# trzy/FasterRCNN

Measured on AMD Instinct MI355X. Metric: images/sec (600x1000) Faster-RCNN VGG-16 inference, higher is better.
Workload: dtype f32 (float32 tensors and accumulation; 15 GEMM layers in the f32x3 split-operand emulation = two fp16 terms per block-scaled operand, three fp16 MFMAs per product; 0 in f32x6 = three bf16 terms, six bf16 MFMAs; the other 2 on exact-f32 MFMA; strict exact-f32 everywhere: config.strict_f32_images_per_

## Files before the change

### fasterrcnn_amd/_native.py

```python
import ctypes as C
import os

_HERE = os.path.dirname(os.path.abspath(__file__))
LIB_PATH = os.environ.get("FRCNN_LIB_PATH") or os.path.join(_HERE, "csrc", "libfrcnn_hip.so")

OK = 0
ABI_VERSION = 21
ERRORS = {0: "FRCNN_OK", -1: "FRCNN_EINVAL", -2: "FRCNN_EHIP", -3: "FRCNN_ENOMEM",
          -4: "FRCNN_EUNSUPPORTED", -5: "FRCNN_ENODEVICE"}
RELU = 1
POOL2 = 2
NUM_KCLASS = 11
KCLASS_NAMES = ("conv3x3_mfma", "conv3x3_c3", "linear_mfma", "proposals", "roi_pool", "other", "winograd_transforms",
                "winograd_gemm", "winograd_x6_transforms", "winograd_x6_gemm", "winograd_x3f")

SYMBOLS = (
    "frcnn_abi_version", "frcnn_error_string", "frcnn_last_hip_error", "frcnn_device_count",
    "frcnn_anchors", "frcnn_pack_conv3x3", "frcnn_pack_conv3x3_c3", "frcnn_pack_fc_chw_to_hwc",
    "frcnn_pack_stack_rows", "frcnn_conv3x3_c3", "frcnn_conv3x3_c3_cmax", "frcnn_conv3x3_workspace_bytes", "frcnn_conv3x3_nhwc",
    "frcnn_maxpool2x2_nhwc",
    "frcnn_linear_workspace_bytes", "frcnn_linear", "frcnn_softmax_rows", "frcnn_rpn_proposals",
    "frcnn_nms", "frcnn_roi_pool", "frcnn_roi_pool_x3t", "frcnn_detections", "frcnn_ctx_create", "frcnn_ctx_create_proposals", "frcnn_ctx_destroy",
    "frcnn_ctx_bytes", "frcnn_vgg16_forward", "frcnn_ctx_tensor", "frcnn_ctx_timing_enable",
    "frcnn_ctx_timing_read",
    "frcnn_output_block_layout", "frcnn_stream_depend", "frcnn_ctx_submit_stats", "frcnn_predict_submit", "frcnn_streams_share_queue",
# ... 1 lines not shown
    "frcnn_maxpool3x3_s2_nhwc", "frcnn_spatial_mean_nhwc", "frcnn_resnet_forward", "frcnn_rpn_targets",
    "frcnn_preprocess_workspace_bytes", "frcnn_preprocess",
    "frcnn_conv3x3_uses_winograd", "frcnn_resnet_block_uses_winograd", "frcnn_pack_conv3x3_winograd",
    "frcnn_pack_conv3x3_winograd_taps", "frcnn_conv3x3_winograd_workspace_bytes",
    "frcnn_conv3x3_nhwc_winograd",
    "frcnn_conv3x3_uses_winograd_fused", "frcnn_resnet_block_uses_winograd_fused", "frcnn_pack_conv3x3_winograd_fused", "frcnn_pack_conv3x3_winograd_fused_taps",
    "frcnn_conv3x3_nhwc_winograd_fused",
    "frcnn_roi_align", "frcnn_roi_align_backward",
    "frcnn_x6t_record_bytes", "frcnn_split_rows_x6t", "frcnn_gemm_x6t_workspace_bytes", "frcnn_gemm_x6t", "frcnn_split_pixels_x6t", "frcnn_split_patches3x3_x6t",
    "frcnn_conv3x3_uses_winograd_x6", "frcnn_conv3x3_winograd_x6_pack_bytes", "frcnn_pack_conv3x3_winograd_x6",
    "frcnn_conv3x3_winograd_x6_workspace_bytes", "frcnn_conv3x3_nhwc_winograd_x6",
    "frcnn_pixel_absmax", "frcnn_split_pixels_x3t", "frcnn_split_patches3x3_x3t",
    "frcnn_x3t_blob_bytes", "frcnn_pack_rows_x3t", "frcnn_conv3x3_winograd_x3_pack_bytes", "frcnn_pack_conv3x3_winograd_x3",
    "frcnn_conv3x3_winograd_x3_workspace_bytes", "frcnn_conv3x3_nhwc_winograd_x3",
    "frcnn_conv3x3_winograd_x3_fused_workspace_bytes", "frcnn_conv3x3_nhwc_winograd_x3_fused", "frcnn_conv3x3_nhwc_winograd_x3_chain",
    "frcnn_x3t_record_bytes", "frcnn_rows_scale_x3t", "frcnn_split_rows_x3t", "frcnn_gemm_x3t_workspace_bytes", "frcnn_gemm_x3t",
    "frcnn_conv3x3_nhwc_winograd_fused_maps", "frcnn_ctx_create_backbone", "frcnn_resnet_backbone", "frcnn_resnet_forward_features", "frcnn_resnet_rpn_roipool", "frcnn_ctx_create_head", "frcnn_resnet_head",
    "frcnn_label_proposals", "frcnn_gather_rows", "frcnn_rpn_loss", "frcnn_detector_loss",
    "frcnn_gemm_tn_math", "frcnn_conv3x3_wgrad_math", "frcnn_conv_wgrad_math", "frcnn_bottleneck_backward_workspace_bytes", "frcnn_bottleneck_backward",
    "frcnn_gemm_tn_workspace_bytes", "frcnn_gemm_tn", "frcnn_conv3x3_wgrad_workspace_bytes", "frcnn_conv3x3_wgrad",
    "frcnn_pack_conv3x3_dgrad", "frcnn_relu_backward", "frcnn_dropout", "frcnn_dropout_relu_backward", "frcnn_add_inplace", "frcnn_maxpool2x2_backward",
    "frcnn_roi_pool_backward_workspace_bytes", "frcnn_roi_pool_backward", "frcnn_transpose", "frcnn_sgd_step", "frcnn_sgd_step_fold",
    "frcnn_conv_wgrad_workspace_bytes", "frcnn_conv_wgrad", "frcnn_conv_dgrad_workspace_bytes", "frcnn_conv_dgrad", "frcnn_conv_dgrad_math",
    "frcnn_pack_conv_dgrad", "frcnn_scale_rows", "frcnn_bn_scale_shift", "frcnn_spatial_mean_backward",
    "frcnn_ops_roi_align", "frcnn_ops_roi_align_backward", "frcnn_ops_roi_pool", "frcnn_ops_roi_pool_backward",
    "frcnn_ops_nms_workspace_bytes", "frcnn_ops_nms",
    "frcnn_ops_ms_roi_align", "frcnn_ops_ms_roi_align_workspace_bytes", "frcnn_ops_ms_roi_align_backward",
    "frcnn_ops_half_run", "frcnn_ops_roi_align_16", "frcnn_ops_roi_align_backward_16", "frcnn_ops_roi_pool_16",
    "frcnn_ops_roi_pool_backward_16", "frcnn_ops_ms_roi_align_16", "frcnn_ops_ms_roi_align_backward_16",
    "frcnn_ops_ps_roi_pool", "frcnn_ops_ps_roi_pool_backward", "frcnn_ops_ps_roi_align", "frcnn_ops_ps_roi_align_backward",
    "frcnn_ops_ps_roi_pool_16", "frcnn_ops_ps_roi_pool_backward_16", "frcnn_ops_ps_roi_align_16", "frcnn_ops_ps_roi_align_backward_16",
# ... 259 lines not shown
    "frcnn_split_pixels_x3t": (C.c_int, [_vp, _vp, _vp, _vp, _i, _i, _i, _i, _i, _i, _vp]),
    "frcnn_split_patches3x3_x3t": (C.c_int, [_vp, _vp, _vp, _vp, _i, _i, _i, _i, _i, _i, _vp]),
    "frcnn_x3t_blob_bytes": (C.c_size_t, [_i, _i, _i]),
    "frcnn_pack_rows_x3t": (C.c_int, [_vp, _i, _sz, _vp, _i, _i, _i, _i, _vp]),
    "frcnn_conv3x3_winograd_x3_pack_bytes": (C.c_size_t, [_i, _i]),
    "frcnn_pack_conv3x3_winograd_x3": (C.c_int, [_vp, _vp, _i, _i, _vp]),
    "frcnn_conv3x3_winograd_x3_workspace_bytes": (C.c_size_t, [_i, _i, _i, _i, _i]),
    "frcnn_conv3x3_nhwc_winograd_x3": (C.c_int, [_vp, _vp, _vp, _vp, _i, _i, _i, _i, _i, _u, _vp, _sz, _vp]),
    "frcnn_conv3x3_winograd_x3_fused_workspace_bytes": (C.c_size_t, [_i, _i, _i]),
    "frcnn_conv3x3_nhwc_winograd_x3_fused": (C.c_int, [_vp, _vp, _vp, _vp, _i, _i, _i, _i, _i, _u, _vp, _sz, _vp]),
    "frcnn_conv3x3_nhwc_winograd_x3_chain": (C.c_int, [_vp, _vp, _vp, _vp, _i, _i, _i, _i, _i, _u, _i, _vp, _sz, _vp, _vp, _vp]),
    "frcnn_x3t_record_bytes": (C.c_size_t, [_i, _i]),
    "frcnn_rows_scale_x3t": (C.c_int, [_vp, _i, _sz, _vp, _i, _i, _i, _i, _vp]),
    "frcnn_split_rows_x3t": (C.c_int, [_vp, _i, _sz, _vp, _vp, _i, _i, _i, _i, _vp]),
    "frcnn_gemm_x3t_workspace_bytes": (C.c_size_t, [_i, _i, _i, _i]),
    "frcnn_gemm_x3t": (C.c_int, [_vp, _vp, _i, _sz, _sz, _vp, _vp, _i, _sz, _sz, _vp, _vp, _vp, _i, _sz, _i, _i, _i, _i, _u, _vp, _sz, _vp]),
    "frcnn_ctx_create_backbone": (C.c_int, [C.POINTER(C.c_void_p), _i, _i, _i]),
    "frcnn_ctx_create_head": (C.c_int, [C.POINTER(C.c_void_p), _i]),
    "frcnn_resnet_rpn_roipool": (C.c_int, [_vp, C.POINTER(ResNetWeights), C.POINTER(ForwardParams), _vp, _i, _i, _vp, _vp, _vp, _vp, _vp, _vp]),
    "frcnn_resnet_head": (C.c_int, [_vp, C.POINTER(ResNetWeights), C.POINTER(ForwardParams), _vp, _i, _vp, _vp, _vp]),
    "frcnn_conv3x3_nhwc_winograd_fused_maps": (C.c_int, [_vp, _vp, _vp, _vp, _i, _i, _i, _i, _i, _u, _vp]),
    "frcnn_label_proposals": (C.c_int, [_vp, _vp, _i, _vp, _vp, _i, _i, _f, _f, C.POINTER(C.c_float), C.POINTER(C.c_float),
                                        _vp, _vp, _vp, _vp, _vp, _vp]),
    "frcnn_gather_rows": (C.c_int, [_vp, _vp, _i, _i, _vp, _vp]),
    "frcnn_rpn_loss": (C.c_int, [_vp, _i, _i, _vp, _i, _vp, _vp, _vp, _vp]),
    "frcnn_detector_loss": (C.c_int, [_vp, _vp, _vp, _vp, _i, _i, _vp, _vp, _i, _vp]),
    "frcnn_gemm_tn_workspace_bytes": (C.c_size_t, [_i, _i, _i]),
    "frcnn_gemm_tn": (C.c_int, [_vp, _i, _vp, _i, _vp, _i, _i, _i, _i, _vp, _sz, _vp]),
    "frcnn_gemm_tn_math": (C.c_int, [_vp, _i, _vp, _i, _vp, _i, _i, _i, _i, _i, _vp, _sz, _vp]),
    "frcnn_conv3x3_wgrad_math": (C.c_int, [_vp, _vp, _vp, _i, _i, _i, _i, _i, _vp, _sz, _vp]),
# ... 104 lines not shown
```

### fasterrcnn_amd/csrc/api.hip

```cpp
#include "common.h"
#include <algorithm>
#include <cmath>
#include <cstring>
#include <string>
#include <vector>
#include <new>

namespace frcnn {

static thread_local std::string g_hip_error;
void set_hip_error(hipError_t e) { g_hip_error = hipGetErrorString(e); }

static size_t align_up(size_t v, size_t a) { return (v + a - 1) / a * a; }

struct EventRec { int cls; hipEvent_t start, stop; };

}

using namespace frcnn;

struct frcnn_ctx {
    int max_h = 0, max_w = 0, max_rois = 0, max_images = 0;
    int max_fh = 0, max_fw = 0, a_cap = 0, pre_cap = 0;
    void* slab = nullptr;
// ... 265 lines not shown
                         void* stream)
{
    if (!d_a || !d_inv_scale) return FRCNN_EINVAL;
    return launch_rows_scale_x3t(d_a, lda, a_batch_floats, d_inv_scale, rows, rows_padded, K, batches, as_stream(stream));
}

int frcnn_split_rows_x3t(const float* d_a, int lda, size_t a_batch_floats, const float* d_inv_scale, void* d_rec, int rows, int rows_padded,
                         int K, int batches, void* stream)
{
    if (!d_a || !d_rec || !d_inv_scale) return FRCNN_EINVAL;
    return launch_split_rows_x3t(d_a, lda, a_batch_floats, d_inv_scale, d_rec, rows, rows_padded, K, batches, as_stream(stream));
}

size_t frcnn_gemm_x3t_workspace_bytes(int M, int N, int K, int batches) { return gemm_x3t_workspace_bytes(M, N, K, batches); }

int frcnn_gemm_x3t(const void* d_a_rec, const float* d_a_inv, int a_rows, size_t a_batch_bytes, size_t a_inv_batch_floats,
                   const void* d_b_rec, const float* d_b_inv, int b_rows, size_t b_batch_bytes, size_t b_inv_batch_floats,
                   const float* d_bias, const float* d_residual, float* d_c, int ldc, size_t c_batch_floats, int M, int N, int K,
                   int batches, unsigned flags, void* d_ws, size_t ws_bytes, void* stream)
{
    return launch_gemm_x3t(d_a_rec, d_a_inv, a_rows, a_batch_bytes, a_inv_batch_floats, d_b_rec, d_b_inv, b_rows, b_batch_bytes,
                           b_inv_batch_floats, d_bias, d_residual, d_c, ldc, c_batch_floats, M, N, K, batches, flags, d_ws, ws_bytes,
                           as_stream(stream));
}

size_t frcnn_conv3x3_winograd_x3_fused_workspace_bytes(int n_maps, int H, int W)
{
    return n_maps > 0 && H > 0 && W > 0 ? conv3x3_winograd_x3_fused_workspace_bytes(n_maps, H, W) : 0;
}

int frcnn_conv3x3_nhwc_winograd_x3_fused(const float* d_x, const void* d_blob, const float* d_bias, float* d_y, int n_maps, int H, int W,
                                         int cin, int cout, unsigned flags, void* d_ws, size_t ws_bytes, void* stream)
{
    if (!d_x || !d_blob || !d_bias || !d_y) return FRCNN_EINVAL;
    return launch_conv3x3_winograd_x3_fused(d_x, d_blob, d_bias, d_y, n_maps, H, W, cin, cout, flags, d_ws, ws_bytes, as_stream(stream));
}

int frcnn_pixel_absmax(const float* d_x, float* d_cmax, long long pixels, int c, void* stream)
// ... 1038 lines not shown
    if (fc_x6t || fc_x3t) { rc = ensure_fc_records(c, s); if (rc) return rc; }
    if (fc_x3t) {
        const int rr = c->rec_rows;
        const size_t w1rec = x3t_record_bytes(4096, 49 * 512), w2rec = x3t_record_bytes(4096, 4096);
        const float* w1inv = reinterpret_cast<const float*>(reinterpret_cast<const unsigned char*>(w->fc1_w) + w1rec);
        const float* w2inv = reinterpret_cast<const float*>(reinterpret_cast<const unsigned char*>(w->fc2_w) + w2rec);
        if (p->roi_op == FRCNN_ROI_ALIGN) {
            STEP(4, launch_roi_align(c->fm, fh, fw, 512, d_props, d_counts + 2, R_, 7, 1.0f / 16.0f, p->roi_sampling_ratio, 0, c->roi_out, s));
            STEP(2, launch_rows_scale_x3t(c->roi_out, 49 * 512, 0, c->roi_inv, R_, rr, 49 * 512, 1, s));
            STEP(2, launch_split_rows_x3t(c->roi_out, 49 * 512, 0, c->roi_inv, c->roi_rec, R_, rr, 49 * 512, 1, s));
        } else {
            STEP(4, launch_roi_pool_x3t(c->fm, fh, fw, 512, d_props, d_counts + 2, R_, 7, 1.0f / 16.0f,
                                        fm_cmax_ready ? const_cast<float*>(fm_cmax_ready) : c->fm_cmax, c->roi_inv, c->roi_rec, rr, s, fm_cmax_ready != nullptr));
        }
        STEP(2, launch_gemm_x3t(c->roi_rec, c->roi_inv, rr, 0, 0, w->fc1_w, w1inv, 4096, 0, 0, w->fc1_b, nullptr, c->fc1_out, 4096, 0, R_, 4096,
                                49 * 512, 1, R, c->lin_ws, c->lin_ws_bytes, s, 0));
        STEP(2, launch_rows_scale_x3t(c->fc1_out, 4096, 0, c->fc1_inv, R_, rr, 4096, 1, s));
        STEP(2, launch_split_rows_x3t(c->fc1_out, 4096, 0, c->fc1_inv, c->fc1_rec, R_, rr, 4096, 1, s));
        STEP(2, launch_gemm_x3t(c->fc1_rec, c->fc1_inv, rr, 0, 0, w->fc2_w, w2inv, 4096, 0, 0, w->fc2_b, nullptr, c->fc2_out, 4096, 0, R_, 4096,
                                4096, 1, R, c->lin_ws, c->lin_ws_bytes, s, 2));
    } else
    if (fc_x6t) {
        const int rr = c->rec_rows;
        if (p->roi_op == FRCNN_ROI_ALIGN) {
            STEP(4, launch_roi_align(c->fm, fh, fw, 512, d_props, d_counts + 2, R_, 7, 1.0f / 16.0f, p->roi_sampling_ratio, 0, c->roi_out, s));
            STEP(2, launch_split_rows_x6t(c->roi_out, 49 * 512, 0, c->roi_rec, R_, rr, 49 * 512, 1, s));
        } else {
            STEP(4, launch_roi_pool_x6t(c->fm, fh, fw, 512, d_props, d_counts + 2, R_, 7, 1.0f / 16.0f, c->roi_rec, rr, s));
        }
        static const int fc_tiles = []() { const char* e = frcnn_knob("FRCNN_FC_TILES"); return e ? atoi(e) : 0; }();
        STEP(2, launch_gemm_x6t(c->roi_rec, rr, 0, w->fc1_w, 4096, 0, w->fc1_b, nullptr, c->fc1_out, 4096, 0, R_, 4096, 49 * 512, 1, R,
                                c->lin_ws, c->lin_ws_bytes, s, fc_tiles));
        STEP(2, launch_split_rows_x6t(c->fc1_out, 4096, 0, c->fc1_rec, R_, rr, 4096, 1, s));
        STEP(2, launch_gemm_x6t(c->fc1_rec, rr, 0, w->fc2_w, 4096, 0, w->fc2_b, nullptr, c->fc2_out, 4096, 0, R_, 4096, 4096, 1, R,
                                c->lin_ws, c->lin_ws_bytes, s, fc_tiles));
// ... 649 lines not shown
```

### fasterrcnn_amd/csrc/common.h

```cpp
#pragma once
#include <hip/hip_runtime.h>
#include <stdint.h>
#include <stddef.h>
#include <stdlib.h>
#include "../../include/frcnn_hip.h"

typedef float f32x4  __attribute__((ext_vector_type(4)));
typedef float f32x16 __attribute__((ext_vector_type(16)));

inline const char* frcnn_knob(const char* name)
{
#ifdef FRCNN_EXPERIMENT_KNOBS
    return getenv(name);
#else
    (void)name;
    return nullptr;
#endif
}

namespace frcnn {

void set_hip_error(hipError_t e);

inline int check_launch() {
// ... 115 lines not shown
int launch_gemm_x6t_reduce(const float* ws, const float* bias, const float* residual, float* c, int ldc, size_t c_batch_floats, int M, int N,
                           int batches, int splits, int relu, hipStream_t s);
size_t x3t_record_bytes(int rows_padded, int K);
int launch_rows_scale_x3t(const float* a, int lda, size_t a_batch_floats, float* inv_scale, int R, int rows_padded, int K, int batches,
                          hipStream_t s);
int launch_split_rows_x3t(const float* a, int lda, size_t a_batch_floats, const float* inv_scale, void* rec, int R, int rows_padded, int K,
                          int batches, hipStream_t s);
int launch_split_pixels_x3t(const float* x, const float* cmax, void* rec, float* inv, int N, int H, int W, int C, int stride, int rows_padded,
                            hipStream_t s);
int launch_split_patches3x3_x3t(const float* x, const float* cmax, void* rec, float* inv, int N, int H, int W, int C, int stride,
                                int rows_padded, hipStream_t s);
size_t gemm_x3t_workspace_bytes(int M, int N, int K, int batches);
int launch_gemm_x3t(const void* a_rec, const float* a_inv, int a_rows, size_t a_batch_bytes, size_t a_inv_batch, const void* b_rec,
                    const float* b_inv, int b_rows, size_t b_batch_bytes, size_t b_inv_batch, const float* bias, const float* residual,
                    float* c, int ldc, size_t c_batch_floats, int M, int N, int K, int batches, unsigned flags, void* ws, size_t ws_bytes,
                    hipStream_t s, int tiles_mode = -1);
size_t x3t_blob_bytes(int rows_padded, int K, int batches);
int launch_pack_rows_x3t(const float* a, int lda, size_t a_batch_floats, void* blob, int R, int rows_padded, int K, int batches, hipStream_t s);
int launch_pixel_absmax(const float* x, float* cmax, long long pixels, int C, hipStream_t s);
size_t conv3x3_winograd_x3_pack_bytes(int cout, int cin);
int launch_pack_conv3x3_winograd_x3(const float* u_f32, void* ublob, int cout, int cin, hipStream_t s);
size_t conv3x3_winograd_x3_workspace_bytes(int N, int H, int W, int cin, int cout);
int winograd_x3_plan(int N, int H, int W, int cin, int cout, unsigned flags, void* ws, size_t ws_bytes, void** V, float** vinv, float** cmax,
                     float** M, void** G, size_t* g_bytes);
int launch_winograd_x3_input(const float* x, float* cmax, void* vrec, float* vinv, int N, int H, int W, int cin, hipStream_t s,
                             const float* cmax_ready = nullptr);
int launch_winograd_x3_gemm(const void* vrec, const float* vinv, const void* ublob, float* M, int N, int H, int W, int cin, int cout, void* gws,
                            size_t gws_bytes, hipStream_t s);
int launch_conv3x3_winograd_x3(const float* x, const void* ublob, const float* b, float* y, int N, int H, int W, int cin, int cout,
                               unsigned flags, void* ws, size_t ws_bytes, hipStream_t s,
                               const float* cmax_ready = nullptr, float* cmax_out = nullptr);
// ... 106 lines not shown
```

### fasterrcnn_amd/csrc/gemm_x3t.hip

```cpp
#include "x3t.h"

namespace frcnn {

typedef _Float16 hx_f16x8 __attribute__((ext_vector_type(8)));

#ifndef HX_ABLATE
#define HX_ABLATE 0
#endif
__global__ __launch_bounds__(256)
void rows_scale_x3t_kernel(const float* __restrict__ a, int lda, size_t a_batch, float* __restrict__ inv_scale, int R, int rows_padded,
                           int K, int batches)
{
    const int lane = threadIdx.x & 63;
    const long long wave = (long long)blockIdx.x * 4 + (threadIdx.x >> 6);
    if (wave >= (long long)batches * rows_padded) return;
    const int row = (int)(wave % rows_padded), batch = (int)(wave / rows_padded);
    float mx = 0.f;
    if (row < R) {
        const float* src = a + (size_t)batch * a_batch + (size_t)row * lda;
        for (int k = 4 * lane; k < K; k += 256) {
            const f32x4 v = *reinterpret_cast<const f32x4*>(src + k);
            mx = fmaxf(fmaxf(mx, fmaxf(fabsf(v[0]), fabsf(v[1]))), fmaxf(fabsf(v[2]), fabsf(v[3])));
        }
    }
// ... 168 lines not shown
    const unsigned char* b;
    const float* a_inv;
    const float* b_inv;
    float* c;
    float* ws;
    const float* bias;
    const float* residual;
    size_t a_batch, b_batch, c_batch;
    size_t a_inv_batch, b_inv_batch;
    int a_rbt, b_rbt;
    int M, N, ldc;
    int nchunks, chunks_per_split, splits, batches;
    int mtiles, ntiles;
    int relu;
    int total;
};

template <int WTM, int WTN, int WVM, int WVN, int NSUB>
struct HxCfg {
    static constexpr int NW = WVM * WVN, THREADS = 64 * NW;
    static constexpr int ARB = WVM * WTM, BRB = WVN * WTN;
    static constexpr int BM = 32 * ARB, BN = 32 * BRB;
    static constexpr int A_BYTES = ARB * HX_RB, B_BYTES = BRB * HX_RB;
    static constexpr int STAGE1 = A_BYTES + B_BYTES;
    static constexpr int STAGE = NSUB * STAGE1;
    static constexpr int NBUF = NSUB == 1 ? 3 : 2;
    static constexpr int DIST = NBUF - 1;
    static constexpr size_t LDS_BYTES = NBUF * (size_t)STAGE;
    static constexpr int NPA = ARB * 2, NPB = BRB * 2, NP = NPA + NPB;
    static constexpr int PPW = (NSUB * NP + NW - 1) / NW;
};

typedef __attribute__((address_space(3))) void* hx_lds_ptr;

template <int WTM, int WTN, int WVM, int WVN, int NSUB>
__global__ __launch_bounds__(64 * WVM * WVN, 2)
void gemm_x3t_kernel(const HxParams p)
{
    using C = HxCfg<WTM, WTN, WVM, WVN, NSUB>;
    extern __shared__ __attribute__((aligned(16))) unsigned char smem_hx[];
    const int tid = threadIdx.x, lane = tid & 63;
    const int wave = __builtin_amdgcn_readfirstlane(tid >> 6);
    const int wm = wave / WVN, wn = wave % WVN;

    int bid = blockIdx.x;
    {
        const int q = p.total >> 3, r = p.total & 7, xcd = bid & 7, idx = bid >> 3;
        bid = (xcd < r ? xcd * (q + 1) : r * (q + 1) + (xcd - r) * q) + idx;
    }
    const int nt = bid % p.ntiles;
    int t = bid / p.ntiles;
    const int mt = t % p.mtiles;
    t /= p.mtiles;
// ... 10 lines not shown
    const unsigned char* bg = p.b + (size_t)batch * p.b_batch + (size_t)nt * C::B_BYTES + (size_t)c_begin * b_chunk + lane * 16;

    auto issue_stage = [&](int s, int buf) {
        const unsigned char* as = ag + (size_t)s * NSUB * a_chunk;
        const unsigned char* bs = bg + (size_t)s * NSUB * b_chunk;
        unsigned char* ldsb = smem_hx + buf * C::STAGE;
#pragma unroll
        for (int i = 0; i < C::PPW; ++i) {
            int q = wave + C::NW * i;
            q = q < NSUB * C::NP ? q : NSUB * C::NP - 1;
            const int sub = q / C::NP, r = q - sub * C::NP;
            const unsigned char* src = r < C::NPA ? as + sub * a_chunk + r * HX_PIECE : bs + sub * b_chunk + (r - C::NPA) * HX_PIECE;
            __builtin_amdgcn_global_load_lds(src, (hx_lds_ptr)(ldsb + sub * C::STAGE1 + r * HX_PIECE), 16, 0, 0);
        }
    };
    f32x16 acc[WTM][WTN];
#pragma unroll
    for (int i = 0; i < WTM; ++i)
#pragma unroll
        for (int j = 0; j < WTN; ++j)
#pragma unroll
            for (int r = 0; r < 16; ++r) acc[i][j][r] = 0.f;

    hx_f16x8 ah[WTM], al[WTM], bh[WTN], bl[WTN];
#pragma unroll
    for (int i = 0; i < WTM; ++i)
#pragma unroll
        for (int e = 0; e < 8; ++e) al[i][e] = (_Float16)0.f;
#pragma unroll
    for (int j = 0; j < WTN; ++j)
#pragma unroll
        for (int e = 0; e < 8; ++e) bh[j][e] = (_Float16)0.f;

#ifndef HX_NO_SCHED
#define HX_NO_SCHED 0
#endif
#define HX_SGB(mask, n) __builtin_amdgcn_sched_group_barrier(mask, n, 0)
#define HX_TERM(A, B)                                                                                  \
    _Pragma("unroll") for (int i = 0; i < WTM; ++i)                                                     \
        _Pragma("unroll") for (int j = 0; j < WTN; ++j)                                                 \
            if (!(HX_ABLATE & 2)) acc[i][j] = __builtin_amdgcn_mfma_f32_32x32x16_f16(B[j], A[i], acc[i][j], 0, 0, 0);

#ifdef HX_CLOCKS
    unsigned long long clk0 = 0, real0 = 0, clk1 = 0, real1 = 0;
    const unsigned long long real_entry = __builtin_amdgcn_s_memrealtime();
#endif
    if (nst > 0) {
        issue_stage(0, 0);
        if (C::DIST == 2) issue_stage(nst > 1 ? 1 : 0, 1);
        asm volatile("s_waitcnt vmcnt(%0)" ::"n"((C::DIST - 1) * C::PPW) : "memory");
        __builtin_amdgcn_s_barrier();
        int cur = 0;
        const int a_off = wm * WTM * HX_RB + lane * 16;
        const int b_off = C::A_BYTES + wn * WTN * HX_RB + lane * 16;
#ifdef HX_CLOCKS
        clk0 = __builtin_readcyclecounter(); real0 = __builtin_amdgcn_s_memrealtime();
#endif
        for (int s = 0; s < nst; ++s) {
            const int nxt = C::NBUF == 3 ? (cur == 0 ? 2 : cur - 1) : (cur ^ 1);
#pragma unroll
            for (int sub = 0; sub < NSUB; ++sub) {
// ... 43 lines not shown
        HX_TERM(al, bh)
        asm volatile("s_waitcnt vmcnt(0)" ::: "memory");
    }
#undef HX_TERM
#undef HX_SGB

    const bool direct = p.splits == 1;
    float* dst;
    int ldd;
    if (direct) { dst = p.c + (size_t)batch * p.c_batch; ldd = p.ldc; }
    else        { dst = p.ws + ((size_t)split * p.batches + batch) * (size_t)p.M * p.N; ldd = p.N; }
    const int m_base = mt * C::BM + 32 * WTM * wm + (lane & 31);
    const int n_base = nt * C::BN + 32 * WTN * wn + 4 * (lane >> 5);
    const float* ainv = p.a_inv + (size_t)batch * p.a_inv_batch;
    const float* binv = p.b_inv + (size_t)batch * p.b_inv_batch;
#pragma unroll
    for (int i = 0; i < WTM; ++i) {
        const int m = m_base + 32 * i;
        if (m >= p.M) continue;
        const float sa = ainv[m];
        float* row = dst + (size_t)m * ldd;
#pragma unroll
        for (int j = 0; j < WTN; ++j) {
#pragma unroll
            for (int g = 0; g < 4; ++g) {
                const int n = n_base + 32 * j + 8 * g;
                if (n >= p.N) continue;
                const f32x4 sb = *reinterpret_cast<const f32x4*>(binv + n);
                f32x4 v;
#pragma unroll
                for (int e = 0; e < 4; ++e) v[e] = (acc[i][j][4 * g + e] * sa) * sb[e];
                if (direct && p.bias != nullptr) v = v + *reinterpret_cast<const f32x4*>(p.bias + n);
                if (direct && p.residual != nullptr)
                    v = v + *reinterpret_cast<const f32x4*>(p.residual + (size_t)batch * p.c_batch + (size_t)m * ldd + n);
                if (direct && p.relu) {
#pragma unroll
                    for (int e = 0; e < 4; ++e) v[e] = fmaxf(v[e], 0.f);
                }
                if (HX_ABLATE & 4) asm volatile("" ::"v"(v));
                else *reinterpret_cast<f32x4*>(row + n) = v;
            }
        }
    }
#ifdef HX_CLOCKS
    if (lane == 0 && p.ws != nullptr) {
        const unsigned long long real_exit = __builtin_amdgcn_s_memrealtime();
        float* o = p.ws + ((size_t)blockIdx.x * C::NW + wave) * 8;
        o[0] = (float)(clk1 - clk0); o[1] = (float)(real1 - real0); o[2] = (float)(real0 - real_entry); o[3] = (float)(real_exit - real1);
        o[4] = (float)nst; o[5] = (float)(real_entry & 0xFFFFFF); o[6] = (float)(real_exit & 0xFFFFFF); o[7] = 1.0f;
    }
#endif
}

size_t x3t_record_bytes(int rows_padded, int K) { return (size_t)(K / 16) * (rows_padded / 32) * HX_RB; }

int launch_rows_scale_x3t(const float* a, int lda, size_t a_batch_floats, float* inv_scale, int R, int rows_padded, int K, int batches,
                          hipStream_t s)
// ... 81 lines not shown
    return pl;
}

size_t gemm_x3t_workspace_bytes(int M, int N, int K, int batches)
{
    if (!gemm_x6t_shape_ok(M, N, K, batches)) return 0;
    size_t need = 0;
    for (int mode = 0; mode < 3; ++mode) {
        const HxPlan pl = plan_gemm_x3t(M, N, K, batches, mode);
        const size_t b = pl.splits > 1 ? (size_t)pl.splits * batches * M * N * sizeof(float) : 0;
        if (b > need) need = b;
    }
    return need;
}

int launch_gemm_x3t(const void* a_rec, const float* a_inv, int a_rows, size_t a_batch_bytes, size_t a_inv_batch, const void* b_rec,
                    const float* b_inv, int b_rows, size_t b_batch_bytes, size_t b_inv_batch, const float* bias, const float* residual,
                    float* c, int ldc, size_t c_batch_floats, int M, int N, int K, int batches, unsigned flags, void* ws, size_t ws_bytes,
                    hipStream_t s, int tiles_mode)
{
    if (!gemm_x6t_shape_ok(M, N, K, batches)) return FRCNN_EUNSUPPORTED;
    if (!a_rec || !b_rec || !a_inv || !b_inv || !c || a_rows % 320 != 0 || a_rows < M || b_rows % 256 != 0 || b_rows < N || ldc < N ||
        ldc % 4 != 0)
        return FRCNN_EINVAL;
    const HxPlan pl = plan_gemm_x3t(M, N, K, batches, tiles_mode);
    if (pl.splits > 1 && (ws == nullptr || ws_bytes < (size_t)pl.splits * batches * M * N * sizeof(float))) return FRCNN_EINVAL;
    HxParams p;
    p.a = static_cast<const unsigned char*>(a_rec);
    p.b = static_cast<const unsigned char*>(b_rec);
    p.a_inv = a_inv; p.b_inv = b_inv;
    p.c = c;
    p.ws = static_cast<float*>(ws);
    p.bias = bias;
    p.residual = residual;
    p.a_batch = a_batch_bytes; p.b_batch = b_batch_bytes; p.c_batch = c_batch_floats;
    p.a_inv_batch = a_inv_batch; p.b_inv_batch = b_inv_batch;
    p.a_rbt = a_rows / 32; p.b_rbt = b_rows / 32;
    p.M = M; p.N = N; p.ldc = ldc;
    p.nchunks = K / 16; p.chunks_per_split = pl.chunks_per_split; p.splits = pl.splits; p.batches = batches;
    p.mtiles = pl.mtiles; p.ntiles = pl.ntiles;
    p.relu = (flags & FRCNN_RELU) ? 1 : 0;
    const long long total = (long long)pl.mtiles * pl.ntiles * batches * pl.splits;
    if (total > 0x7fffffffLL) return FRCNN_EINVAL;
    p.total = (int)total;
    static const int env_nsub = []() { const char* e = frcnn_knob("FRCNN_HX_NSUB"); return e ? atoi(e) : 0; }();
    const int last = p.nchunks - (pl.splits - 1) * pl.chunks_per_split;
    const bool even = pl.chunks_per_split % 2 == 0 && last % 2 == 0;
    const int nsub = !even ? 1 : (env_nsub == 1 || env_nsub == 2) ? env_nsub : (pl.chunks_per_split >= 64 ? 2 : 1);
#define HX_LAUNCH(TM, TN, VM, VN, NS)                                                                          \
    do {                                                                                                      \
        using C = HxCfg<TM, TN, VM, VN, NS>;                                                                    \
        auto kern = gemm_x3t_kernel<TM, TN, VM, VN, NS>;                                                        \
        FRCNN_MAX_LDS_ONCE(kern, C::LDS_BYTES);                                                                 \
        hipLaunchKernelGGL(kern, dim3((unsigned)total), dim3(C::THREADS), C::LDS_BYTES, s, p);                  \
    } while (0)
    if (pl.cfg == 1) { if (nsub == 2) HX_LAUNCH(5, 1, 1, 4, 2); else HX_LAUNCH(5, 1, 1, 4, 1); }
    else             { if (nsub == 2) HX_LAUNCH(5, 2, 2, 4, 2); else HX_LAUNCH(5, 2, 2, 4, 1); }
#undef HX_LAUNCH
    int rc = check_launch();
    if (rc || pl.splits == 1) return rc;
    return launch_gemm_x6t_reduce(static_cast<const float*>(ws), bias, residual, c, ldc, c_batch_floats, M, N, batches, pl.splits, p.relu, s);
}

}
```

### include/frcnn_hip.h

```cpp
#ifndef FRCNN_HIP_H
#define FRCNN_HIP_H

#include <stddef.h>
#include <stdint.h>

#ifdef __cplusplus
extern "C" {
#endif

#define FRCNN_OK            0
#define FRCNN_EINVAL       -1
#define FRCNN_EHIP         -2
#define FRCNN_ENOMEM       -3
#define FRCNN_EUNSUPPORTED -4
#define FRCNN_ENODEVICE    -5

#define FRCNN_ABI_VERSION 21

#define FRCNN_RELU   1u
#define FRCNN_POOL2  2u
#define FRCNN_X3G_WSPLIT 0x800u

int         frcnn_abi_version(void);
const char* frcnn_error_string(int code);
const char* frcnn_last_hip_error(void);
int         frcnn_device_count(void);

int frcnn_anchors(int image_h, int image_w, int fh, int fw, int feature_pixels,
                  float* d_anchor_map, float* d_valid_map, void* stream);

size_t frcnn_preprocess_workspace_bytes(int H, int W, int out_h, int out_w);
int frcnn_preprocess(const unsigned char* d_rgb, int H, int W, int out_h, int out_w, int bgr_order,
                     int horizontal_flip, float scaling, const float* means, const float* stds,
                     float* d_out, unsigned char* d_out_u8, void* d_ws, size_t ws_bytes, void* stream);

// ... 61 lines not shown
int frcnn_conv3x3_nhwc_winograd_x3_fused(const float* d_x, const void* d_blob, const float* d_bias, float* d_y, int n_maps, int H, int W,
                                         int cin, int cout, unsigned flags, void* d_ws, size_t ws_bytes, void* stream);
int frcnn_conv3x3_nhwc_winograd_x3_chain(const float* d_x, const void* d_blob, const float* d_bias, float* d_y, int n_maps, int H, int W, int cin,
                                         int cout, unsigned flags, int one_launch, void* d_ws, size_t ws_bytes, const float* d_cmax_in,
                                         float* d_cmax_out, void* stream);
size_t frcnn_x3t_record_bytes(int rows_padded, int K);
int frcnn_rows_scale_x3t(const float* d_a, int lda, size_t a_batch_floats, float* d_inv_scale, int rows, int rows_padded, int K, int batches,
                         void* stream);
int frcnn_split_rows_x3t(const float* d_a, int lda, size_t a_batch_floats, const float* d_inv_scale, void* d_rec, int rows, int rows_padded,
                         int K, int batches, void* stream);
size_t frcnn_gemm_x3t_workspace_bytes(int M, int N, int K, int batches);
int frcnn_gemm_x3t(const void* d_a_rec, const float* d_a_inv, int a_rows, size_t a_batch_bytes, size_t a_inv_batch_floats,
                   const void* d_b_rec, const float* d_b_inv, int b_rows, size_t b_batch_bytes, size_t b_inv_batch_floats,
                   const float* d_bias, const float* d_residual, float* d_c, int ldc, size_t c_batch_floats, int M, int N, int K,
                   int batches, unsigned flags, void* d_ws, size_t ws_bytes, void* stream);

int frcnn_split_pixels_x6t(const float* d_x, void* d_rec, int N, int H, int W, int C, int stride, int rows_padded, void* stream);
int frcnn_conv3x3_uses_winograd_x6(int cin, int cout);
size_t frcnn_conv3x3_winograd_x6_pack_bytes(int cout, int cin);
int frcnn_pack_conv3x3_winograd_x6(const float* d_w_oihw, const float* d_row_scale, void* d_u_rec, int cout, int cin, void* stream);
size_t frcnn_conv3x3_winograd_x6_workspace_bytes(int n_maps, int H, int W, int cin, int cout);
int frcnn_conv3x3_nhwc_winograd_x6(const float* d_x, const void* d_u_rec, const float* d_bias, float* d_y, int n_maps, int H, int W, int cin,
                                   int cout, unsigned flags, void* d_ws, size_t ws_bytes, void* stream);
int frcnn_split_patches3x3_x6t(const float* d_x, void* d_rec, int N, int H, int W, int C, int stride, int rows_padded, void* stream);
int frcnn_maxpool2x2_nhwc(const float* d_x, float* d_y, int H, int W, int c, void* stream);

int frcnn_fold_bn_pack(const float* d_w_oihw, const float* d_gamma, const float* d_beta,
                       const float* d_mean, const float* d_var, float eps, int cout, int cin, int ksize,
                       float* d_w_packed, float* d_b_packed, void* stream);
size_t frcnn_conv_workspace_bytes(int N, int H, int W, int cin, int cout, int ksize, int stride, int pad);
// ... 399 lines not shown
```

Measured before the change: 979.6.

## Add 16x16x32 MFMA variant of x3t GEMM with padded-tile skipping for fc1

Adds a templated path to the split-fp16 x3t GEMM kernel that uses 16x16x32 f16 MFMA instructions with per-16-row accumulators instead of the 32x32 shape. When the row count leaves the last 16-row tile of a wave empty, that tile's loads and MFMAs are skipped. The path is enabled by default for the fc1 head GEMM. fc2 keeps the old shape. The aim is to cut MFMA work wasted on padded ROI rows and possibly raise instruction throughput, at the cost of more LDS reads and a different register footprint. A plan-query API and env override are also added.

```diff
diff --git a/fasterrcnn_amd/_native.py b/fasterrcnn_amd/_native.py
--- a/fasterrcnn_amd/_native.py
+++ b/fasterrcnn_amd/_native.py
@@ -9,6 +9,7 @@
 ERRORS = {0: "FRCNN_OK", -1: "FRCNN_EINVAL", -2: "FRCNN_EHIP", -3: "FRCNN_ENOMEM",
           -4: "FRCNN_EUNSUPPORTED", -5: "FRCNN_ENODEVICE"}
 RELU = 1
+X3T_MFMA16, X3T_MFMA16_PADDED = 0x1000, 0x2000
 POOL2 = 2
 NUM_KCLASS = 11
 KCLASS_NAMES = ("conv3x3_mfma", "conv3x3_c3", "linear_mfma", "proposals", "roi_pool", "other", "winograd_transforms",
@@ -40,7 +41,7 @@
     "frcnn_x3t_blob_bytes", "frcnn_pack_rows_x3t", "frcnn_conv3x3_winograd_x3_pack_bytes", "frcnn_pack_conv3x3_winograd_x3",
     "frcnn_conv3x3_winograd_x3_workspace_bytes", "frcnn_conv3x3_nhwc_winograd_x3",
     "frcnn_conv3x3_winograd_x3_fused_workspace_bytes", "frcnn_conv3x3_nhwc_winograd_x3_fused", "frcnn_conv3x3_nhwc_winograd_x3_chain",
-    "frcnn_x3t_record_bytes", "frcnn_rows_scale_x3t", "frcnn_split_rows_x3t", "frcnn_gemm_x3t_workspace_bytes", "frcnn_gemm_x3t",
+    "frcnn_x3t_record_bytes", "frcnn_rows_scale_x3t", "frcnn_split_rows_x3t", "frcnn_gemm_x3t_workspace_bytes", "frcnn_gemm_x3t", "frcnn_gemm_x3t_plan",
     "frcnn_conv3x3_nhwc_winograd_fused_maps", "frcnn_ctx_create_backbone", "frcnn_resnet_backbone", "frcnn_resnet_forward_features", "frcnn_resnet_rpn_roipool", "frcnn_ctx_create_head", "frcnn_resnet_head",
     "frcnn_label_proposals", "frcnn_gather_rows", "frcnn_rpn_loss", "frcnn_detector_loss",
     "frcnn_gemm_tn_math", "frcnn_conv3x3_wgrad_math", "frcnn_conv_wgrad_math", "frcnn_bottleneck_backward_workspace_bytes", "frcnn_bottleneck_backward",
@@ -330,6 +331,7 @@
     "frcnn_rows_scale_x3t": (C.c_int, [_vp, _i, _sz, _vp, _i, _i, _i, _i, _vp]),
     "frcnn_split_rows_x3t": (C.c_int, [_vp, _i, _sz, _vp, _vp, _i, _i, _i, _i, _vp]),
     "frcnn_gemm_x3t_workspace_bytes": (C.c_size_t, [_i, _i, _i, _i]),
+    "frcnn_gemm_x3t_plan": (C.c_int, [_i, _i, _i, _i, _u, _vp]),
     "frcnn_gemm_x3t": (C.c_int, [_vp, _vp, _i, _sz, _sz, _vp, _vp, _i, _sz, _sz, _vp, _vp, _vp, _i, _sz, _i, _i, _i, _i, _u, _vp, _sz, _vp]),
     "frcnn_ctx_create_backbone": (C.c_int, [C.POINTER(C.c_void_p), _i, _i, _i]),
     "frcnn_ctx_create_head": (C.c_int, [C.POINTER(C.c_void_p), _i]),
diff --git a/fasterrcnn_amd/csrc/api.hip b/fasterrcnn_amd/csrc/api.hip
--- a/fasterrcnn_amd/csrc/api.hip
+++ b/fasterrcnn_amd/csrc/api.hip
@@ -303,6 +303,10 @@
 
 size_t frcnn_gemm_x3t_workspace_bytes(int M, int N, int K, int batches) { return gemm_x3t_workspace_bytes(M, N, K, batches); }
 
+static constexpr int FC1_X3T_SHAPE = 1, FC2_X3T_SHAPE = 0;
+
+static int x3t_shape_of_flags(unsigned flags) { return (flags & FRCNN_X3T_MFMA16) ? ((flags & FRCNN_X3T_MFMA16_PADDED) ? 2 : 1) : 0; }
+
 int frcnn_gemm_x3t(const void* d_a_rec, const float* d_a_inv, int a_rows, size_t a_batch_bytes, size_t a_inv_batch_floats,
                    const void* d_b_rec, const float* d_b_inv, int b_rows, size_t b_batch_bytes, size_t b_inv_batch_floats,
                    const float* d_bias, const float* d_residual, float* d_c, int ldc, size_t c_batch_floats, int M, int N, int K,
@@ -310,7 +314,12 @@
 {
     return launch_gemm_x3t(d_a_rec, d_a_inv, a_rows, a_batch_bytes, a_inv_batch_floats, d_b_rec, d_b_inv, b_rows, b_batch_bytes,
                            b_inv_batch_floats, d_bias, d_residual, d_c, ldc, c_batch_floats, M, N, K, batches, flags, d_ws, ws_bytes,
-                           as_stream(stream));
+                           as_stream(stream), -1, x3t_shape_of_flags(flags));
+}
+
+int frcnn_gemm_x3t_plan(int M, int N, int K, int batches, unsigned flags, int32_t* out7)
+{
+    return gemm_x3t_plan(M, N, K, batches, x3t_shape_of_flags(flags), -1, out7);
 }
 
 size_t frcnn_conv3x3_winograd_x3_fused_workspace_bytes(int n_maps, int H, int W)
@@ -1379,11 +1388,11 @@
                                         fm_cmax_ready ? const_cast<float*>(fm_cmax_ready) : c->fm_cmax, c->roi_inv, c->roi_rec, rr, s, fm_cmax_ready != nullptr));
         }
         STEP(2, launch_gemm_x3t(c->roi_rec, c->roi_inv, rr, 0, 0, w->fc1_w, w1inv, 4096, 0, 0, w->fc1_b, nullptr, c->fc1_out, 4096, 0, R_, 4096,
-                                49 * 512, 1, R, c->lin_ws, c->lin_ws_bytes, s, 0));
+                                49 * 512, 1, R, c->lin_ws, c->lin_ws_bytes, s, 0, FC1_X3T_SHAPE));
         STEP(2, launch_rows_scale_x3t(c->fc1_out, 4096, 0, c->fc1_inv, R_, rr, 4096, 1, s));
         STEP(2, launch_split_rows_x3t(c->fc1_out, 4096, 0, c->fc1_inv, c->fc1_rec, R_, rr, 4096, 1, s));
         STEP(2, launch_gemm_x3t(c->fc1_rec, c->fc1_inv, rr, 0, 0, w->fc2_w, w2inv, 4096, 0, 0, w->fc2_b, nullptr, c->fc2_out, 4096, 0, R_, 4096,
-                                4096, 1, R, c->lin_ws, c->lin_ws_bytes, s, 2));
+                                4096, 1, R, c->lin_ws, c->lin_ws_bytes, s, 2, FC2_X3T_SHAPE));
     } else
     if (fc_x6t) {
         const int rr = c->rec_rows;
diff --git a/fasterrcnn_amd/csrc/common.h b/fasterrcnn_amd/csrc/common.h
--- a/fasterrcnn_amd/csrc/common.h
+++ b/fasterrcnn_amd/csrc/common.h
@@ -153,7 +153,8 @@
 int launch_gemm_x3t(const void* a_rec, const float* a_inv, int a_rows, size_t a_batch_bytes, size_t a_inv_batch, const void* b_rec,
                     const float* b_inv, int b_rows, size_t b_batch_bytes, size_t b_inv_batch, const float* bias, const float* residual,
                     float* c, int ldc, size_t c_batch_floats, int M, int N, int K, int batches, unsigned flags, void* ws, size_t ws_bytes,
-                    hipStream_t s, int tiles_mode = -1);
+                    hipStream_t s, int tiles_mode = -1, int shape = 0);
+int gemm_x3t_plan(int M, int N, int K, int batches, int shape, int tiles_mode, int out[7]);
 size_t x3t_blob_bytes(int rows_padded, int K, int batches);
 int launch_pack_rows_x3t(const float* a, int lda, size_t a_batch_floats, void* blob, int R, int rows_padded, int K, int batches, hipStream_t s);
 int launch_pixel_absmax(const float* x, float* cmax, long long pixels, int C, hipStream_t s);
diff --git a/fasterrcnn_amd/csrc/gemm_x3t.hip b/fasterrcnn_amd/csrc/gemm_x3t.hip
--- a/fasterrcnn_amd/csrc/gemm_x3t.hip
+++ b/fasterrcnn_amd/csrc/gemm_x3t.hip
@@ -206,6 +206,7 @@
     int mtiles, ntiles;
     int relu;
     int total;
+    int skip_tiles;
 };
 
 template <int WTM, int WTN, int WVM, int WVN, int NSUB>
@@ -225,10 +226,11 @@
 
 typedef __attribute__((address_space(3))) void* hx_lds_ptr;
 
-template <int WTM, int WTN, int WVM, int WVN, int NSUB>
+template <int WTM, int WTN, int WVM, int WVN, int NSUB, int MF = 0>
 __global__ __launch_bounds__(64 * WVM * WVN, 2)
 void gemm_x3t_kernel(const HxParams p)
 {
+    static_assert(MF == 0 || NSUB == 2, "the 16x16x32 shape consumes two 16-k chunks per instruction");
     using C = HxCfg<WTM, WTN, WVM, WVN, NSUB>;
     extern __shared__ __attribute__((aligned(16))) unsigned char smem_hx[];
     const int tid = threadIdx.x, lane = tid & 63;
@@ -269,23 +271,34 @@
             __builtin_amdgcn_global_load_lds(src, (hx_lds_ptr)(ldsb + sub * C::STAGE1 + r * HX_PIECE), 16, 0, 0);
         }
     };
-    f32x16 acc[WTM][WTN];
-#pragma unroll
-    for (int i = 0; i < WTM; ++i)
-#pragma unroll
-        for (int j = 0; j < WTN; ++j)
+    constexpr int RT = 2 * WTM, CT = 2 * WTN;
+    f32x16 acc[MF ? 1 : WTM][MF ? 1 : WTN];
+    f32x4 acc4[MF ? RT : 1][MF ? CT : 1];
+#pragma unroll
+    for (int i = 0; i < (MF ? 1 : WTM); ++i)
+#pragma unroll
+        for (int j = 0; j < (MF ? 1 : WTN); ++j)
 #pragma unroll
             for (int r = 0; r < 16; ++r) acc[i][j][r] = 0.f;
-
-    hx_f16x8 ah[WTM], al[WTM], bh[WTN], bl[WTN];
-#pragma unroll
-    for (int i = 0; i < WTM; ++i)
+#pragma unroll
+    for (int i = 0; i < (MF ? RT : 1); ++i)
+#pragma unroll
+        for (int j = 0; j < (MF ? CT : 1); ++j)
+#pragma unroll
+            for (int r = 0; r < 4; ++r) acc4[i][j][r] = 0.f;
+
+    constexpr int TG = CT >= 4 ? 1 : 2, NG = RT / TG;
+    static_assert(RT % TG == 0, "row tiles per step");
+    hx_f16x8 ah[MF ? 2 * TG : WTM], al[MF ? 2 * TG : WTM], bh[MF ? CT : WTN], bl[MF ? CT : WTN];
+#pragma unroll
+    for (int i = 0; i < (MF ? 2 * TG : WTM); ++i)
 #pragma unroll
         for (int e = 0; e < 8; ++e) al[i][e] = (_Float16)0.f;
 #pragma unroll
-    for (int j = 0; j < WTN; ++j)
+    for (int j = 0; j < (MF ? CT : WTN); ++j)
 #pragma unroll
         for (int e = 0; e < 8; ++e) bh[j][e] = (_Float16)0.f;
+    const bool last_live = !p.skip_tiles || mt * C::BM + 32 * WTM * wm + 16 * (RT - 1) < p.M;
 
 #ifndef HX_NO_SCHED
 #define HX_NO_SCHED 0
@@ -300,6 +313,69 @@
     unsigned long long clk0 = 0, real0 = 0, clk1 = 0, real1 = 0;
     const unsigned long long real_entry = __builtin_amdgcn_s_memrealtime();
 #endif
+    if constexpr (MF == 1) {
+        if (nst > 0) {
+            issue_stage(0, 0);
+            asm volatile("s_waitcnt vmcnt(0)" ::: "memory");
+            __builtin_amdgcn_s_barrier();
+            int cur = 0;
+            const int frag = ((lane >> 5) & 1) * C::STAGE1 + ((lane >> 4) & 1) * 512 + (lane & 15) * 16;
+            const int a_off = wm * WTM * HX_RB + frag;
+            const int b_off = C::A_BYTES + wn * WTN * HX_RB + frag;
+#ifdef HX_CLOCKS
+            clk0 = __builtin_readcyclecounter(); real0 = __builtin_amdgcn_s_memrealtime();
+#endif
+#define HX_LD16(base, t, term) (*reinterpret_cast<const hx_f16x8*>((base) + ((t) >> 1) * HX_RB + ((t) & 1) * 256 + (term) * HX_PIECE))
+#define HX_READA(rt) do { ah[(rt) % (2 * TG)] = HX_LD16(at, rt, 0); al[(rt) % (2 * TG)] = HX_LD16(at, rt, 1); } while (0)
+#define HX_TILE16(rt)                                                                                                                      \
+    do {                                                                                                                                   \
+        _Pragma("unroll") for (int j = 0; j < CT; ++j)                                                                                     \
+            acc4[rt][j] = __builtin_amdgcn_mfma_f32_16x16x32_f16(bh[j], al[(rt) % (2 * TG)], acc4[rt][j], 0, 0, 0);                   \
+        _Pragma("unroll") for (int j = 0; j < CT; ++j)                                                                                     \
+            acc4[rt][j] = __builtin_amdgcn_mfma_f32_16x16x32_f16(bl[j], ah[(rt) % (2 * TG)], acc4[rt][j], 0, 0, 0);                   \
+        _Pragma("unroll") for (int j = 0; j < CT; ++j)                                                                                     \
+            acc4[rt][j] = __builtin_amdgcn_mfma_f32_16x16x32_f16(bh[j], ah[(rt) % (2 * TG)], acc4[rt][j], 0, 0, 0);                   \
+    } while (0)
+            for (int s = 0; s < nst; ++s) {
+                const unsigned char* at = smem_hx + cur * C::STAGE + a_off;
+                const unsigned char* bt = smem_hx + cur * C::STAGE + b_off;
+#pragma unroll
+                for (int j = 0; j < CT; ++j) bh[j] = HX_LD16(bt, j, 0);
+#pragma unroll
+                for (int t = 0; t < TG; ++t) HX_READA(t);
+#pragma unroll
+                for (int j = 0; j < CT; ++j) bl[j] = HX_LD16(bt, j, 1);
+                issue_stage(s + 1 < nst ? s + 1 : nst - 1, cur ^ 1);
+                __builtin_amdgcn_sched_barrier(0);
+#pragma unroll
+                for (int gi = 0; gi < NG; ++gi) {
+                    if (gi + 1 < NG) {
+#pragma unroll
+                        for (int t = 0; t < TG; ++t) {
+                            const int rt = (gi + 1) * TG + t;
+                            if (rt < RT - 1 || last_live) HX_READA(rt);
+                        }
+                    }
+#pragma unroll
+                    for (int t = 0; t < TG; ++t) {
+                        const int rt = gi * TG + t;
+                        if (rt < RT - 1 || last_live) HX_TILE16(rt);
+                    }
+                    __builtin_amdgcn_sched_barrier(0);
+                }
+                asm volatile("s_waitcnt vmcnt(0) lgkmcnt(0)" ::: "memory");
+                __builtin_amdgcn_s_barrier();
+                cur ^= 1;
+                __builtin_amdgcn_sched_barrier(0);
+            }
+#undef HX_TILE16
+#undef HX_READA
+#undef HX_LD16
+#ifdef HX_CLOCKS
+            clk1 = __builtin_readcyclecounter(); real1 = __builtin_amdgcn_s_memrealtime();
+#endif
+        }
+    } else
     if (nst > 0) {
         issue_stage(0, 0);
         if (C::DIST == 2) issue_stage(nst > 1 ? 1 : 0, 1);
@@ -373,6 +449,34 @@
     const int n_base = nt * C::BN + 32 * WTN * wn + 4 * (lane >> 5);
     const float* ainv = p.a_inv + (size_t)batch * p.a_inv_batch;
     const float* binv = p.b_inv + (size_t)batch * p.b_inv_batch;
+    if constexpr (MF == 1) {
+        const int m16 = mt * C::BM + 32 * WTM * wm + (lane & 15);
+        const int n16 = nt * C::BN + 32 * WTN * wn + 4 * (lane >> 4);
+#pragma unroll
+        for (int i = 0; i < RT; ++i) {
+            const int m = m16 + 16 * i;
+            if (m >= p.M) continue;
+            const float sa = ainv[m];
+            float* row = dst + (size_t)m * ldd;
+#pragma unroll
+            for (int j = 0; j < CT; ++j) {
+                const int n = n16 + 16 * j;
+                if (n >= p.N) continue;
+                const f32x4 sb = *reinterpret_cast<const f32x4*>(binv + n);
+                f32x4 v;
+#pragma unroll
+                for (int e = 0; e < 4; ++e) v[e] = (acc4[i][j][e] * sa) * sb[e];
+                if (direct && p.bias != nullptr) v = v + *reinterpret_cast<const f32x4*>(p.bias + n);
+                if (direct && p.residual != nullptr)
+                    v = v + *reinterpret_cast<const f32x4*>(p.residual + (size_t)batch * p.c_batch + (size_t)m * ldd + n);
+                if (direct && p.relu) {
+#pragma unroll
+                    for (int e = 0; e < 4; ++e) v[e] = fmaxf(v[e], 0.f);
+                }
+                *reinterpret_cast<f32x4*>(row + n) = v;
+            }
+        }
+    } else {
 #pragma unroll
     for (int i = 0; i < WTM; ++i) {
         const int m = m_base + 32 * i;
@@ -400,6 +504,7 @@
                 else *reinterpret_cast<f32x4*>(row + n) = v;
             }
         }
+    }
     }
 #ifdef HX_CLOCKS
     if (lane == 0 && p.ws != nullptr) {
@@ -511,10 +616,35 @@
     return need;
 }
 
+struct HxPick { int nsub, shape; };
+
+static HxPick pick_gemm_x3t(const HxPlan& pl, int nchunks, int shape)
+{
+    static const int env_nsub = []() { const char* e = frcnn_knob("FRCNN_HX_NSUB"); return e ? atoi(e) : 0; }();
+    static const int env_shape = []() { const char* e = frcnn_knob("FRCNN_HX_SHAPE"); return e ? atoi(e) : -1; }();
+    if (env_shape >= 0 && env_shape <= 2) shape = env_shape;
+    const int last = nchunks - (pl.splits - 1) * pl.chunks_per_split;
+    const bool even = pl.chunks_per_split % 2 == 0 && last % 2 == 0;
+    HxPick pk;
+    pk.shape = even && (shape == 1 || shape == 2) ? shape : 0;
+    pk.nsub = !even ? 1 : pk.shape ? 2 : (env_nsub == 1 || env_nsub == 2) ? env_nsub : (pl.chunks_per_split >= 64 ? 2 : 1);
+    return pk;
+}
+
+int gemm_x3t_plan(int M, int N, int K, int batches, int shape, int tiles_mode, int out[7])
+{
+    if (!gemm_x6t_shape_ok(M, N, K, batches)) return FRCNN_EUNSUPPORTED;
+    if (!out) return FRCNN_EINVAL;
+    const HxPlan pl = plan_gemm_x3t(M, N, K, batches, tiles_mode);
+    const HxPick pk = pick_gemm_x3t(pl, K / 16, shape);
+    out[0] = pl.cfg; out[1] = pl.mtiles; out[2] = pl.ntiles; out[3] = pl.splits; out[4] = pl.chunks_per_split; out[5] = pk.nsub; out[6] = pk.shape;
+    return FRCNN_OK;
+}
+
 int launch_gemm_x3t(const void* a_rec, const float* a_inv, int a_rows, size_t a_batch_bytes, size_t a_inv_batch, const void* b_rec,
                     const float* b_inv, int b_rows, size_t b_batch_bytes, size_t b_inv_batch, const float* bias, const float* residual,
                     float* c, int ldc, size_t c_batch_floats, int M, int N, int K, int batches, unsigned flags, void* ws, size_t ws_bytes,
-                    hipStream_t s, int tiles_mode)
+                    hipStream_t s, int tiles_mode, int shape)
 {
     if (!gemm_x6t_shape_ok(M, N, K, batches)) return FRCNN_EUNSUPPORTED;
     if (!a_rec || !b_rec || !a_inv || !b_inv || !c || a_rows % 320 != 0 || a_rows < M || b_rows % 256 != 0 || b_rows < N || ldc < N ||
@@ -540,19 +670,17 @@
     const long long total = (long long)pl.mtiles * pl.ntiles * batches * pl.splits;
     if (total > 0x7fffffffLL) return FRCNN_EINVAL;
     p.total = (int)total;
-    static const int env_nsub = []() { const char* e = frcnn_knob("FRCNN_HX_NSUB"); return e ? atoi(e) : 0; }();
-    const int last = p.nchunks - (pl.splits - 1) * pl.chunks_per_split;
-    const bool even = pl.chunks_per_split % 2 == 0 && last % 2 == 0;
-    const int nsub = !even ? 1 : (env_nsub == 1 || env_nsub == 2) ? env_nsub : (pl.chunks_per_split >= 64 ? 2 : 1);
-#define HX_LAUNCH(TM, TN, VM, VN, NS)                                                                          \
+    const HxPick pk = pick_gemm_x3t(pl, p.nchunks, shape);
+    p.skip_tiles = pk.shape == 1 ? 1 : 0;
+#define HX_LAUNCH(TM, TN, VM, VN, NS, MF)                                                                      \
     do {                                                                                                      \
         using C = HxCfg<TM, TN, VM, VN, NS>;                                                                    \
-        auto kern = gemm_x3t_kernel<TM, TN, VM, VN, NS>;                                                        \
+        auto kern = gemm_x3t_kernel<TM, TN, VM, VN, NS, MF>;                                                    \
         FRCNN_MAX_LDS_ONCE(kern, C::LDS_BYTES);                                                                 \
         hipLaunchKernelGGL(kern, dim3((unsigned)total), dim3(C::THREADS), C::LDS_BYTES, s, p);                  \
     } while (0)
-    if (pl.cfg == 1) { if (nsub == 2) HX_LAUNCH(5, 1, 1, 4, 2); else HX_LAUNCH(5, 1, 1, 4, 1); }
-    else             { if (nsub == 2) HX_LAUNCH(5, 2, 2, 4, 2); else HX_LAUNCH(5, 2, 2, 4, 1); }
+    if (pl.cfg == 1) { if (pk.shape) HX_LAUNCH(5, 1, 1, 4, 2, 1); else if (pk.nsub == 2) HX_LAUNCH(5, 1, 1, 4, 2, 0); else HX_LAUNCH(5, 1, 1, 4, 1, 0); }
+    else             { if (pk.shape) HX_LAUNCH(5, 2, 2, 4, 2, 1); else if (pk.nsub == 2) HX_LAUNCH(5, 2, 2, 4, 2, 0); else HX_LAUNCH(5, 2, 2, 4, 1, 0); }
 #undef HX_LAUNCH
     int rc = check_launch();
     if (rc || pl.splits == 1) return rc;
diff --git a/include/frcnn_hip.h b/include/frcnn_hip.h
--- a/include/frcnn_hip.h
+++ b/include/frcnn_hip.h
@@ -19,6 +19,8 @@
 
 #define FRCNN_RELU   1u
 #define FRCNN_POOL2  2u
+#define FRCNN_X3T_MFMA16 0x1000u
+#define FRCNN_X3T_MFMA16_PADDED 0x2000u
 #define FRCNN_X3G_WSPLIT 0x800u
 
 int         frcnn_abi_version(void);
@@ -110,6 +112,7 @@
                    const void* d_b_rec, const float* d_b_inv, int b_rows, size_t b_batch_bytes, size_t b_inv_batch_floats,
                    const float* d_bias, const float* d_residual, float* d_c, int ldc, size_t c_batch_floats, int M, int N, int K,
                    int batches, unsigned flags, void* d_ws, size_t ws_bytes, void* stream);
+int frcnn_gemm_x3t_plan(int M, int N, int K, int batches, unsigned flags, int32_t* out7);
 
 int frcnn_split_pixels_x6t(const float* d_x, void* d_rec, int N, int H, int W, int C, int stride, int rows_padded, void* stream);
 int frcnn_conv3x3_uses_winograd_x6(int cin, int cout);
```

Result: no change. 987.6, median of 6 (+0.8%).
